# xuangu-fang/Gaussian-Process-Slover-for-High-Freq-PDE

Hardware: AMD Instinct MI355X
Metric: log-joint iters/sec + fp64 Cholesky GFLOP/s, 2D Poisson 256^2, 1-8 GPU (higher is better)
Workload: dtype f64; 1 GPU; C4: 2D Poisson 256x256 Kronecker grid, Matern52_Cos_1d, Q=30, fp64; Q=30, kernel=Matern52_Cos_1d, equation=poisson_2d-sin_sin, parallelism=replicas x1 (one independent problem per GPU)

## Files before the change

### gaussian-process-slover-for-high-freq-pde_amd/csrc/gpk_internal.h

```cpp
#pragma once
#include <vector>
#include <hip/hip_runtime.h>
#include <stdint.h>

namespace gpk {

constexpr int QMAX = 64;
constexpr int PADM = 32;
constexpr int NB = 32;
constexpr double SQRT5 = 2.23606797749978969641;
constexpr double TWO_PI = 6.28318530717958647692;

enum Kind { SE_COS = 0, MATERN52_COS = 1, SE = 2, MATERN52 = 3 };

__host__ __device__ inline bool kind_matern(int k) { return k == MATERN52_COS || k == MATERN52; }
__host__ __device__ inline bool kind_cos(int k) { return k == SE_COS || k == MATERN52_COS; }
inline int pad_up(int n) { return (n + PADM - 1) / PADM * PADM; }

struct AxisConst {
  double w[QMAX];
  double a[QMAX];
  double om[QMAX];
  double oml[QMAX];
};

__host__ __device__ inline double om_low(double freq, double om) { return fma(TWO_PI, freq, -om); }

__device__ __forceinline__ void phase_sincos(double om, double oml, double d, double& S, double& C) {
  const double h = om * d;
  const double l = fma(om, d, -h) + oml * d;
  double s, c;
  sincos(h, &s, &c);
  S = fma(l, c, s);
  C = fma(-l, s, c);
}

template <bool MATERN>
__device__ __forceinline__ double radial_exp(double d, double a, double& r) {
  double l;
  if (MATERN) {
    const double p = SQRT5 * a;
    r = p * d;
    l = fma(p, d, -r) + fma(SQRT5, a, -p) * d;
  } else {
    const double d2 = d * d;
    r = a * d2;
    l = fma(a, d2, -r) + a * fma(d, d, -d2);
  }
  const double E = exp(-r);
  return fma(-l, E, E);
}

struct StepScalars {
  double tau, v;
  double bc1, bc2;
};

template <bool MATERN>
__device__ __forceinline__ void radial(double d, double a, double& m0, double& m1, double& m2) {
  double r;
  const double E = radial_exp<MATERN>(d, a, r);
  if (MATERN) {
    m0 = (1.0 + r + r * r * (1.0 / 3.0)) * E;
    m1 = -(SQRT5 / 3.0) * a * r * (1.0 + r) * E;
    m2 = (5.0 / 3.0) * a * a * (r * r - r - 1.0) * E;
  } else {
    const double d2 = d * d, g = E;
    m0 = g;
    m1 = -2.0 * a * d * g;
    m2 = (4.0 * a * a * d2 - 2.0 * a) * g;
  }
}

template <bool MATERN>
__device__ __forceinline__ void radial_l(double d, double a, double& m0, double& m1, double& m2,
                                         double& m0l, double& m1l, double& m2l) {
  double r;
  const double E = radial_exp<MATERN>(d, a, r);
  if (MATERN) {
    double ka = (SQRT5 / 3.0) * a, k2 = (5.0 / 3.0) * a * a;
    double r2 = r * r;
    m0 = (1.0 + r + r2 * (1.0 / 3.0)) * E;
    m1 = -ka * r * (1.0 + r) * E;
    m2 = k2 * (r2 - r - 1.0) * E;
    m0l = -(r2 * (1.0 / 3.0)) * (1.0 + r) * E;
    m1l = -ka * r * (2.0 + 2.0 * r - r2) * E;
    m2l = k2 * (-r2 * r + 5.0 * r2 - 2.0 * r - 2.0) * E;
  } else {
    const double d2 = d * d, g = E;
    m0 = g;
    m1 = -2.0 * a * d * g;
    m2 = (4.0 * a * a * d2 - 2.0 * a) * g;
    m0l = -a * d2 * g;
    m1l = (-2.0 * a * d + 2.0 * a * a * d2 * d) * g;
    m2l = (10.0 * a * a * d2 - 2.0 * a - 4.0 * a * a * a * d2 * d2) * g;
  }
}

}

namespace gpk {

constexpr int BGAP_CHUNK = 2048, BGAP_PARTS_MAX = 16;
struct PrepArgs {
  const double* params;
  int off_kp[2];
  int off_tau, off_v;
  int naxes, has_cos;
  AxisConst* kc;
  StepScalars* sc;
  int* count;
  int apply;
  double b1, b2;
  const double* Up; const double* bvals; const int* bidx;
  int nb, dim, n1, n2, p2;
  double* bgap;
  int bgap_parts;
  int skip;
  int* snap_count; unsigned int* viol0; int* slot0;
  double* snap; const double* snap_m; const double* snap_v; size_t snap_np;
  unsigned int* nce_flag;
};

constexpr int CLS_VMAX = 32;
struct ClassArgs {
  int ncls;
  int vmax;
  const double* dist;
  const int* cid;
  const int* cbase;
  const unsigned char* vidx;
  double* kval;
  double* dval;
  int nchunk, rb;
  double* part;
};

struct AssembleArgs {
  const double* x;
  int n;
  int p;
  const AxisConst* kc;
  double jitter;
  double* K;
  double* Kc;
  double* D;
  int deriv;
  double* piv; double* ldet; double* pst; int* status;
  unsigned int* flag;
  ClassArgs cls;
};
hipError_t launch_gather_only(const AssembleArgs* a, int naxes, hipStream_t s);
hipError_t launch_assemble(int kind, int q, const AssembleArgs* a, int naxes, const PrepArgs& prep,
                           hipStream_t s, bool eval_only = false);
hipError_t launch_pairs(int kind, int q, const double* x1, const double* x2, long n,
                        const AxisConst* kc, int deriv, double* out, hipStream_t s);
hipError_t launch_cross(int kind, int q, const double* xr, int nr, const double* xc, int nc,
                        int ld, const AxisConst* kc, double jitter, int deriv, double* K,
                        double* D, hipStream_t s);

struct SpdArgs {
  double* X;
  double* Y;
  int p;
  int n;
  double* piv;
  double* ldet;
  double* pst;
  int* status;
  unsigned int* flag;
  int wide;
  int no_quarters;
  int qfirst;
  double* Z;
  const unsigned* sched;
  int sched_paired;
};
int wide_sched_stride(int T2);
void wide_schedule(int T2, bool paired, std::vector<unsigned>& tab);
hipError_t launch_spd_inverse(SpdArgs* args, int nmat, double** final_out, hipStream_t s,
                              bool pivot0_done = false);
hipError_t launch_spd_stage(SpdArgs* args, int nmat, int stage, hipStream_t s);

constexpr int CHAIN_MAX_BLOCKS = 512;
struct ChainArgs {
  double* X; double* PB; double* piv; double* ldet; double* pst; int* status;
  unsigned int* flags;
  int p, n;
  const int* cid; const double* kval; const double* dval; const double* x; double jitter;
  double* Kc; double* D;
  int tu, td;
  const double* Bu; int ldbu, bu_t;
  double* Ou; int ldou, ou_t;
  double* Od; int ldod;
  double* PBa; int ldpba;
  double* gran;
  int lookahead;
  double* PB2; unsigned int* epoch;
};
__host__ __device__ inline size_t multi_half(int p) { return (size_t)p * p + (size_t)32 * p; }
__host__ __device__ inline size_t chain_half(int p, bool multi) { return multi ? multi_half(p) : (size_t)32 * p; }
constexpr unsigned long long CHAIN_SENTINEL = 0x7ff4dead7ff4deadull;
constexpr unsigned int CHAIN_SENTINEL32 = 0x7ff4deadu;
int spd_chain_blocks(const int* p, int nmat, bool aug);
int spd_chain_capacity(int deriv, bool gather);
__host__ __device__ inline int chain_role(int m, int x, int T, int TC) {
  const int nt = T * TC, nc = 2 * (T - 1);
  auto crit = [TC](int i) { return (i & 1) ? ((i >> 1) + 1) * (TC + 1) : (i >> 1) * (TC + 1) + 1; };
  int r;
  if (m == 0) {
    if (x == nt) return nt;
    if (x >= nt - nc) return crit(x - (nt - nc));
    r = x;
  } else {
    if (x == 0) return nt;
    if (x <= nc) return crit(x - 1);
    r = x - 1 - nc;
  }
  int tile = r;
  for (int i = 0; i < nc; ++i)
    if (crit(i) <= tile) ++tile;
  return tile;
}
int spd_chain_multi_blocks(const int* p, int nmat);
int spd_chain_multi_capacity(int deriv, bool gather);
hipError_t launch_spd_chain_multi(const ChainArgs* a, int nmat, int deriv, hipStream_t s,
                                  const PrepArgs* prep = nullptr, int q = 0);
hipError_t launch_spd_chain(const ChainArgs* a, int nmat, int deriv, hipStream_t s,
                            const PrepArgs* prep = nullptr, int q = 0);

constexpr int SPD_BIG_MIN = 1600;
constexpr int SPD_WIDE_MIN = 3072;
size_t spd_big_piv_doubles(int p);
void spd_big_set_workgroups(int g);
constexpr unsigned SPIN_CAP = 1u << 22;
hipError_t wait_limit_spdinv(unsigned polls);
hipError_t wait_limit_spdbig(unsigned polls);
hipError_t wait_limit_assemble(unsigned polls);
hipError_t wait_limit_pgrad(unsigned polls);
hipError_t launch_spd_inverse_big(SpdArgs* args, int nmat, double** final_out, hipStream_t s);
hipError_t launch_spd_big_stage(SpdArgs* args, int nmat, int stage, hipStream_t s, bool mirror = true);
double spd_big_update_flops(const SpdArgs* args, int nmat, int k, bool with_pivot);
hipError_t launch_spd_big_tiles(SpdArgs* args, int nmat, int k, hipStream_t s);
int spd_big_sweeps(int p, int wide);

constexpr double REFINE_COND_LB = 100.0;

enum Epi {
  EPI_STORE = 0,
  EPI_RESID = 1,
  EPI_QUAD = 2,
};
struct GemmDesc {
  const double* A; const double* B; int lda, ldb, ta, tb;
  const double* A2; const double* B2; int lda2, ldb2, ta2, tb2;
  double alpha, alpha2, beta;
  const double* C0; int ldc0;
  double* C; int ldc;
  int M, N, K, K2;
  int epi;
  int ac;
  const double* F; const double* U; int ldf;
  int vscale, vscale2;
  double* red;
  double* red2; const double* Q1; const double* Q2;
  const double* gate; int ngate;
  double* Y; const double* Ys; int ldy;
  int tag;
  const double* Cp; int ldcp;
  double* cpart; const int* bcid; const int* bcbase; const double* bsx; int bn, bncls;
};
__host__ __device__ inline int class_slots(int T) { return 4 * T; }
constexpr int CB_SLOTS = 31 * 8;
constexpr int CB_VMAX = 16;
constexpr int GEMM_MAX_BATCH = 4;
struct GemmBatch {
  GemmDesc d[GEMM_MAX_BATCH];
};
hipError_t launch_gemm_batch(const GemmDesc* descs, int ndesc, int max_tiles,
                             const StepScalars* sc, hipStream_t s, int small);
inline bool gemm_use_small(long tiles16_total) { return tiles16_total <= 16384; }
enum { GEMM_TILED32 = 0, GEMM_SMALL = 1, GEMM_BIG = 2, GEMM_HUGE = 3 };
constexpr long GEMM_HUGE_MIN_TILES = 256;
int gemm_variant(const GemmDesc* descs, int ndesc, int force_big);
int gemm_tiles(const GemmDesc& d, int variant);
hipError_t launch_gemm_auto(const GemmDesc* descs, int ndesc, const StepScalars* sc, hipStream_t s,
                            int variant);

struct SlabGemm {
  const double* A; const double* B; size_t sB;
  double* C; size_t sC;
  const double* C0; size_t sC0;
  int M, N, K, nb;
  double alpha, beta;
};
constexpr int SLAB_TILE64_MIN = 512;
int slab_gemm_tile(const SlabGemm& g);
hipError_t launch_gemm_slab(const SlabGemm& g, hipStream_t s, int tile = 0);

__device__ __forceinline__ bool gate_open(const double* gate) {
  if (!gate) return true;
  const double k00 = gate[0];
  const double mx = __longlong_as_double(*reinterpret_cast<const long long*>(gate + 1));
  return mx * k00 > REFINE_COND_LB;
}

struct GemvDesc {
  const double* A; int lda; const double* x; double* y; int p; int rows;
  double alpha;
  const double* C0; double beta;
  int epi;
  int ac;
  const double* F; const double* U;
  const double* U0;
  double* red;
  double* red2; const double* Q1; const double* Q2;
  const double* gate; int ngate;
  const int* cid; const double* cv; double cdiag; int ident;
};
hipError_t launch_gemv(const GemvDesc& d, hipStream_t s);
int gemv_blocks(int rows);

struct PGradArgs {
  const double* x; int n; int p;
  const AxisConst* kc;
  const double* GK; const double* GD;
  const double* Kinv;
  const double* alpha; const double* beta; const double* R;
  double halfc;
  int deriv;
  double* part;
  double* part_lo;
  ClassArgs cls;
  const double* cpK; const double* cpD; int cslots;
};
struct TailArgs;
hipError_t launch_pgrad(int kind, int q, int mode1d, const PGradArgs* a, int naxes,
                        int blocks_per_axis, const StepScalars* sc, hipStream_t s,
                        const TailArgs* tail = nullptr, int shard_rank = 0, int shard_n = 1);
int pgrad_blocks(int n);
int pgrad_class_blocks(int ncls);

}
```

### gaussian-process-slover-for-high-freq-pde_amd/csrc/pgrad.hip

```cpp
#include <algorithm>

#include "gpk_internal.h"
#include "gpk_trace.h"
#include "fields_dd.h"
#include "spd_pivot.h"
#include "prep_dev.h"

namespace gpk {
GPK_TRACE_TU(pgrad)
GPK_WAIT_LIMIT_SETTER(wait_limit_pgrad)
}
#define FIN_PROBE(slot) TR_HI(slot)
#include "stepk_dev.h"

#ifndef GPK_PG_PAIRS
#define GPK_PG_PAIRS 64
#endif

namespace gpk {

constexpr int PAIRS = GPK_PG_PAIRS;
constexpr int PG_SUB = 1024 / PAIRS;

struct PGradBatch {
  PGradArgs ax[2];
  int tiles[2];
  int naxes, bpa;
  int shard_rank, shard_n;
  TailArgs tail;
};

__device__ __forceinline__ void st_wt(double* p, double v) {
  __hip_atomic_store(p, v, __ATOMIC_RELAXED, __HIP_MEMORY_SCOPE_AGENT);
}

__device__ __forceinline__ bool arrive_last(unsigned int* counter, unsigned int n, int* s_flag) {
  asm volatile("s_waitcnt vmcnt(0)" ::: "memory");
  __syncthreads();
  if (threadIdx.x == 0) {
    const unsigned prev = atomicAdd(counter, 1u);
    *s_flag = prev == n - 1u;
  }
  __syncthreads();
  return *s_flag != 0;
}


__device__ void pgrad_tail(const PGradBatch& b, int axis, int blk, int q) {
  const TailArgs& T = b.tail;
  __shared__ int s_last;
  const int t = threadIdx.x;
  const int gi = blk / T.tg;
  const int gsize = min(T.tg, b.bpa - gi * T.tg);
  if (t == 0 && blk == 0 && axis == 0) TR_HI(SLOT_PG_CONTRACT);
  if (t == 0 && blk == b.bpa - 1 && axis == b.naxes - 1) TR_HI(SLOT_PG_START);
  if (!arrive_last(T.gcount + axis * T.ngpa + gi, (unsigned)gsize, &s_last)) return;
  if (t == 0) {
    TR_LO(SLOT_PG_GARR);
    TR_HI(SLOT_PG_GARR);
  }
  const double* part = b.ax[axis].part;
  const double* part_lo = b.ax[axis].part_lo;
  for (int x = t; x < 3 * QMAX; x += 256) {
    const size_t go = (size_t)(axis * T.ngpa + gi) * (3 * QMAX) + x;
    if (T.gpart_lo) {
      dd::D acc = {0.0, 0.0};
      if ((x % QMAX) < q)
        acc = strided_sum_dd(part + (size_t)gi * T.tg * (3 * QMAX) + x,
                             part_lo + (size_t)gi * T.tg * (3 * QMAX) + x, 3 * QMAX, gsize);
      st_wt(T.gpart + go, acc.h);
      st_wt(T.gpart_lo + go, acc.l);
      continue;
    }
    double acc = 0.0;
    if ((x % QMAX) < q)
      acc = strided_sum(part + (size_t)gi * T.tg * (3 * QMAX) + x, 3 * QMAX, gsize);
    st_wt(T.gpart + go, acc);
  }
  if (t == 0) T.gcount[axis * T.ngpa + gi] = 0u;
  if (t == 0) TR_HI(SLOT_PG_GROUP);
  if (!arrive_last(T.top, (unsigned)(b.naxes * T.ngpa), &s_last)) return;
  if (t == 0) TR_LO(SLOT_PG_TOP);
  if (t == 0) *T.top = 0u;
  if (t == 0) TR_HI(SLOT_PG_TOP);
  finalize_body(T.fin, 2);
  if (t == 0) TR_HI(SLOT_PG_FINAL);
  if (T.nce_flag) {
    asm volatile("s_waitcnt vmcnt(0)" ::: "memory");
    __syncthreads();
    if (t == 0) __hip_atomic_store(T.nce_flag, 1u, __ATOMIC_RELAXED, __HIP_MEMORY_SCOPE_AGENT);
  }
}

template <bool MATERN, bool COS, int DERIV>
__device__ void next_class_values(const PGradBatch& b, int ax, int blk, int q) {
  const ClassArgs& C = b.ax[ax].cls;
  if (blk * 8 >= C.ncls) return;
  __shared__ double sw[QMAX], sa[QMAX], so[QMAX], sol[QMAX];
  const int t = threadIdx.x, u = blk * 8 + (t >> 5);
  const double d = u < C.ncls ? C.dist[u] : 0.0;
  if (t == 0) (void)spin_until_ge<1>(b.tail.nce_flag, 1u, b.tail.nce_status);
  __syncthreads();
  if (t < q) {
    const Layout& L = b.tail.fin.L;
    const double* kp = b.tail.fin.kp_wt + ((ax == 0 ? L.off_kp[0] : L.off_kp[1]) - L.off_small);
    axis_component_v(ld_wt(kp + t), ld_wt(kp + q + t), ld_wt(kp + 2 * q + t), sw[t], sa[t], so[t], sol[t]);
  }
  __syncthreads();
  class_value_store<MATERN, COS, DERIV>(C, u, d, sw, sa, so, sol, q);
}

template <int V, int DERIV, bool MODE1D, bool LDSB = false>
__global__ __launch_bounds__(256) void class_sum_kernel(PGradBatch b,
                                                       const StepScalars* __restrict__ sc, int vb = 0) {
  const int axis = blockIdx.z, band = blockIdx.y, chunk = blockIdx.x;
  const PGradArgs& A = b.ax[axis];
  const ClassArgs& C = A.cls;
  const int n = A.n, p = A.p;
  if (band * 64 >= n || chunk >= C.nchunk) return;
  if (MODE1D && min(n, chunk * C.rb + C.rb) - 1 < band * 64) return;
  const int t = threadIdx.x, lane = t & 63, w = t >> 6;
  if (TR_FIRST) TR_LO(SLOT_CLASS_SUM);
  if (TR_LAST) TR_LO(SLOT_CSUM_START);
  const int k = band * 64 + lane;
  const bool kv = k < n;
  const int cb = kv ? C.cbase[k] : 0;
  const int nvar = kv ? C.cbase[k + 1] - cb : 0;
  const int r0 = chunk * C.rb, r1 = min(n, r0 + C.rb);
  int nvw = V;
  if constexpr (V > 16) {
    nvw = nvar;
#pragma unroll
    for (int o = 32; o > 0; o >>= 1) nvw = max(nvw, __shfl_xor(nvw, o, 64));
    nvw = __builtin_amdgcn_readfirstlane(nvw);
  }
  double ak[LDSB ? 1 : V], ad[LDSB ? 1 : V];
#pragma unroll
  for (int x = 0; x < (LDSB ? 1 : V); ++x) ak[x] = ad[x] = 0.0;
  extern __shared__ double lbin[];
  double* mybin = lbin + (size_t)w * 2 * vb * 64;
  if constexpr (LDSB) {
    for (int x = 0; x < vb; ++x) {
      mybin[x * 64 + lane] = 0.0;
      mybin[(vb + x) * 64 + lane] = 0.0;
    }
  }
  double vs = 0.0, hc = 0.0;
  if (MODE1D) {
    vs = sc->v;
    hc = A.halfc;
  }
  static_assert(!(MODE1D && DERIV == 1), "the 1D fold assumes a symmetric G_D sign");
  constexpr int RP = MODE1D ? 8 : 4, NP = 8;
  for (int base = r0; base < r1; base += 4 * RP) {
    int ii[NP], jj[NP], msk[NP];
    if (MODE1D) {
#pragma unroll
      for (int s = 0; s < NP; ++s) {
        const int r = base + w + 4 * s;
        const bool lo = kv && r < r1 && r >= k;
        ii[s] = lo ? r : 0;
        jj[s] = lo ? r - k : 0;
        msk[s] = -(int)lo;
      }
    } else {
#pragma unroll
      for (int s = 0; s < RP; ++s) {
        const int r = base + w + 4 * s;
        const bool in = kv && r < r1;
        const bool lo = in && r >= k, up = in && k > 0 && r + k < n;
        ii[2 * s] = lo ? r : 0;
        jj[2 * s] = lo ? r - k : 0;
        msk[2 * s] = -(int)lo;
        ii[2 * s + 1] = up ? r : 0;
        jj[2 * s + 1] = up ? r + k : 0;
        msk[2 * s + 1] = -(int)up;
      }
    }
    int cv[NP];
    double g0[NP], g1[NP];
#pragma unroll
    for (int s = 0; s < NP; ++s) cv[s] = C.cid[(size_t)ii[s] * p + jj[s]];
    if (MODE1D) {
      double ai[NP], aj[NP], bi[NP], bj[NP], ri[NP], rj[NP];
#pragma unroll
      for (int s = 0; s < NP; ++s) {
        g0[s] = A.Kinv[(size_t)ii[s] * p + jj[s]];
        ai[s] = A.alpha[ii[s]];
        aj[s] = A.alpha[jj[s]];
        bi[s] = A.beta[ii[s]];
        bj[s] = A.beta[jj[s]];
        ri[s] = A.R[ii[s]];
        rj[s] = A.R[jj[s]];
      }
      if (k == 0) {
#pragma unroll
        for (int s = 0; s < NP; ++s) {
          g1[s] = vs * ri[s] * aj[s];
          g0[s] = hc * g0[s] - 0.5 * ai[s] * aj[s] - vs * bi[s] * aj[s];
        }
      } else {
#pragma unroll
        for (int s = 0; s < NP; ++s) {
          g1[s] = vs * (ri[s] * aj[s] + rj[s] * ai[s]);
          g0[s] = 2.0 * hc * g0[s] - ai[s] * aj[s] - vs * (bi[s] * aj[s] + bj[s] * ai[s]);
        }
      }
    } else {
#pragma unroll
      for (int s = 0; s < NP; ++s) g0[s] = A.GK[(size_t)ii[s] * p + jj[s]];
#pragma unroll
      for (int s = 0; s < NP; ++s) g1[s] = A.GD[(size_t)ii[s] * p + jj[s]];
    }
    if (DERIV == 1) {
      double xi[NP], xj[NP];
#pragma unroll
      for (int s = 0; s < NP; ++s) {
        xi[s] = A.x[ii[s]];
        xj[s] = A.x[jj[s]];
      }
#pragma unroll
      for (int s = 0; s < NP; ++s)
        if (!(xi[s] - xj[s] >= 0.0)) g1[s] = -g1[s];
    }
    if constexpr (LDSB) {
#pragma unroll
      for (int s = 0; s < NP; ++s) {
        const int v = cv[s] - cb;
        if (msk[s] && v >= 0 && v < vb) {
          __hip_atomic_fetch_add(mybin + v * 64 + lane, g0[s], __ATOMIC_RELAXED, __HIP_MEMORY_SCOPE_WORKGROUP);
          __hip_atomic_fetch_add(mybin + (vb + v) * 64 + lane, g1[s], __ATOMIC_RELAXED, __HIP_MEMORY_SCOPE_WORKGROUP);
        }
      }
    } else if constexpr (V > 16) {
      int vv[8];
#pragma unroll
      for (int s = 0; s < 8; ++s) vv[s] = ((cv[s] - cb) & msk[s]) | ~msk[s];
#pragma unroll
      for (int x = 0; x < V; ++x) {
        if (x < nvw) {
#pragma unroll
          for (int s = 0; s < 8; ++s) {
            ak[x] += (vv[s] == x) ? g0[s] : 0.0;
            ad[x] += (vv[s] == x) ? g1[s] : 0.0;
          }
        }
      }
    } else {
#pragma unroll
      for (int s = 0; s < 8; ++s) {
        const int v = ((cv[s] - cb) & msk[s]) | ~msk[s];
#pragma unroll
        for (int x = 0; x < V; ++x) {
          ak[x] += (v == x) ? g0[s] : 0.0;
          ad[x] += (v == x) ? g1[s] : 0.0;
        }
      }
    }
  }
  if constexpr (LDSB) {
    __syncthreads();
    if (w == 0) {
      double* pk = C.part + (size_t)chunk * C.ncls + cb;
      double* pd = C.part + (size_t)(C.nchunk + chunk) * C.ncls + cb;
      for (int x = 0; x < nvar; ++x) {
        double rk = lbin[x * 64 + lane], rd = lbin[(vb + x) * 64 + lane];
#pragma unroll
        for (int ww = 1; ww < 4; ++ww) {
          rk = rk + lbin[(size_t)ww * 2 * vb * 64 + x * 64 + lane];
          rd = rd + lbin[(size_t)ww * 2 * vb * 64 + (vb + x) * 64 + lane];
        }
        pk[x] = rk;
        pd[x] = rd;
      }
    }
    if (TR_FIRST) TR_HI(SLOT_CLASS_SUM);
    if (TR_LAST) TR_HI(SLOT_CSUM_START);
    return;
  }
  __shared__ double red[2][V][64];
#pragma unroll
  for (int ww = 0; ww < 4; ++ww) {
    if (w == ww) {
#pragma unroll
      for (int x = 0; x < V; ++x) {
        if (x < nvw) {
          red[0][x][lane] = ww == 0 ? ak[x] : red[0][x][lane] + ak[x];
          red[1][x][lane] = ww == 0 ? ad[x] : red[1][x][lane] + ad[x];
        }
      }
    }
    __syncthreads();
  }
  if (w == 0) {
    double* pk = C.part + (size_t)chunk * C.ncls + cb;
    double* pd = C.part + (size_t)(C.nchunk + chunk) * C.ncls + cb;
#pragma unroll
    for (int x = 0; x < V; ++x)
      if (x < nvar) {
        pk[x] = red[0][x][lane];
        pd[x] = red[1][x][lane];
      }
  }
  if (TR_FIRST) TR_HI(SLOT_CLASS_SUM);
  if (TR_LAST) TR_HI(SLOT_CSUM_START);
}

constexpr int PG_CLS = 16;

template <bool MATERN, bool COS, int DERIV, bool MODE1D, bool CLS, bool DD = false>
__global__ __launch_bounds__(256) void pgrad_kernel(PGradBatch b, int q,
                                                    const StepScalars* __restrict__ sc) {
  const int axis = blockIdx.y;
  const int blk = blockIdx.x;
  if (TR_FIRST) TR_LO(SLOT_PGRAD);
  if (axis == b.naxes + 1) {
    if (blk == 0) finalize_body(b.tail.fin, 1);
    return;
  }
  if (axis >= b.naxes + 2) {
    if (CLS && b.tail.nce_flag) next_class_values<MATERN, COS, DERIV>(b, axis - (b.naxes + 2), blk, q);
    return;
  }
  if (axis == b.naxes) {
    if (threadIdx.x == 0 && blk == 0) TR_LO(SLOT_PG_UPLANE);
    const int nu = tail_nu(b.tail.adam.L);
    for (int e = blk * 256 + threadIdx.x; e < nu; e += gridDim.x * 256) adam_u_elem(b.tail.adam, e);
    if (threadIdx.x == 0 && blk == 0) TR_HI(SLOT_PG_UPLANE);
    if (threadIdx.x == 0 && blk == gridDim.x - 1) TR_HI(SLOT_PG_ULAST);
    return;
  }
  if (blk >= b.bpa) return;
  const bool trl = threadIdx.x == 0 && blk == b.bpa - 1 && axis == b.naxes - 1;
  if (trl) TR_LO(SLOT_PG_START);
  const PGradArgs& A = b.ax[axis];
  const int tile = CLS ? blk : blk / PG_SUB, chunk = blk % PG_SUB;
  if (CLS ? blk * PG_CLS >= A.cls.ncls : tile >= b.tiles[axis]) {
    if (b.tail.fused) pgrad_tail(b, axis, blk, q);
    return;
  }
  if (b.shard_n > 1 && tile % b.shard_n != b.shard_rank) return;

  __shared__ double sd[PAIRS], swk[PAIRS], swd[PAIRS];
  __shared__ double sw[QMAX], sa[QMAX], so[QMAX], sol[QMAX];
  __shared__ double sacc[8][3][32];
  const int t = threadIdx.x;
  if (t < q) {
    sw[t] = A.kc->w[t];
    sa[t] = A.kc->a[t];
    so[t] = A.kc->om[t];
    sol[t] = A.kc->oml[t];
  }
  constexpr int NP = CLS ? PG_CLS : PAIRS;
  if (CLS) {
    const ClassArgs& C = A.cls;
    const int ul = t & (PG_CLS - 1), cs = t / PG_CLS;
    const int u = blk * PG_CLS + ul;
    double sk = 0.0, sdd = 0.0;
    if (u < C.ncls && A.cpK) {
      for (int e = cs; e < A.cslots; e += 256 / PG_CLS) {
        sk += A.cpK[(size_t)e * C.ncls + u];
        sdd += A.cpD[(size_t)e * C.ncls + u];
      }
    } else if (u < C.ncls) {
      for (int c = cs; c < C.nchunk; c += 256 / PG_CLS) {
        sk += C.part[(size_t)c * C.ncls + u];
        sdd += C.part[(size_t)(C.nchunk + c) * C.ncls + u];
      }
    }
    sacc[cs >> 1][0][(cs & 1) * PG_CLS + ul] = sk;
    sacc[cs >> 1][1][(cs & 1) * PG_CLS + ul] = sdd;
    __syncthreads();
    if (t < PG_CLS) {
      double a = 0.0, d = 0.0;
#pragma unroll
      for (int x = 0; x < 256 / PG_CLS; ++x) {
        a += sacc[x >> 1][0][(x & 1) * PG_CLS + t];
        d += sacc[x >> 1][1][(x & 1) * PG_CLS + t];
      }
      const bool ok = u < C.ncls;
      sd[t] = ok ? C.dist[u] : 0.0;
      swk[t] = ok ? a : 0.0;
      swd[t] = ok ? d : 0.0;
    }
  } else if (t < PAIRS) {
    int I = (int)((sqrt(8.0 * tile + 1.0) - 1.0) * 0.5);
    while ((I + 1) * (I + 2) / 2 <= tile) ++I;
    while (I * (I + 1) / 2 > tile) --I;
    const int J = tile - I * (I + 1) / 2;
    const int i = I * 32 + chunk * (PAIRS / 32) + (t >> 5), j = J * 32 + (t & 31);
    double d = 0.0, wk = 0.0, wd = 0.0;
    if (i < A.n && j < A.n) {
      const double diff = A.x[i] - A.x[j];
      d = fabs(diff);
      const double sij = diff >= 0.0 ? 1.0 : -1.0;
      const double sji = (A.x[j] - A.x[i]) >= 0.0 ? 1.0 : -1.0;
      double gkij, gkji, gdij, gdji;
      if (MODE1D) {
        const double v = sc->v;
        const double ai = A.alpha[i], aj = A.alpha[j];
        gkij = A.halfc * A.Kinv[(size_t)i * A.p + j] - 0.5 * ai * aj - v * A.beta[i] * aj;
        gkji = A.halfc * A.Kinv[(size_t)j * A.p + i] - 0.5 * aj * ai - v * A.beta[j] * ai;
        gdij = v * A.R[i] * aj;
        gdji = v * A.R[j] * ai;
      } else {
        gkij = A.GK[(size_t)i * A.p + j];
        gkji = A.GK[(size_t)j * A.p + i];
        gdij = A.GD[(size_t)i * A.p + j];
        gdji = A.GD[(size_t)j * A.p + i];
      }
      if (DERIV == 1) {
        gdij *= sij;
        gdji *= sji;
      }
      if (I == J) {
        wk = gkij;
        wd = gdij;
      } else {
        wk = gkij + gkji;
        wd = gdij + gdji;
      }
    }
    sd[t] = d;
    swk[t] = wk;
    swd[t] = wd;
  }
  __syncthreads();
  if (TR_FIRST) TR_HI(SLOT_PG_STAGED);

  const int g = t >> 5, ql = t & 31;
  double* out = A.part + (size_t)blk * (3 * QMAX);
  __shared__ double slo[DD ? 8 : 1][3][32];
  for (int q0 = 0; q0 < q; q0 += 32) {
    const int c = q0 + ql;
    double accf = 0.0, accl = 0.0, accw = 0.0;
    dd::D xf = {0.0, 0.0}, xl = {0.0, 0.0}, xw = {0.0, 0.0};
    if (c < q) {
      const double a = sa[c], om = so[c], oml = sol[c];
      for (int e = g; e < NP; e += 8) {
        const double wk = swk[e], wd = swd[e];
        if (wk == 0.0 && wd == 0.0) continue;
        const double d = sd[e];
        if constexpr (DD) {
          dd::D fw, fl, ff, dw, dl, df;
          fields_dd<MATERN, COS, DERIV>(d, a, om, oml, fw, fl, ff, dw, dl, df);
          xw = dd::add(xw, dd::add(dd::mul_d(fw, wk), dd::mul_d(dw, wd)));
          xl = dd::add(xl, dd::add(dd::mul_d(fl, wk), dd::mul_d(dl, wd)));
          xf = dd::add(xf, dd::add(dd::mul_d(ff, wk), dd::mul_d(df, wd)));
          continue;
        }
        double m0, m1, m2, m0l, m1l, m2l;
        radial_l<MATERN>(d, a, m0, m1, m2, m0l, m1l, m2l);
        if (COS) {
          double S, C;
          phase_sincos(om, oml, d, S, C);
          const double c0 = C, c1 = -om * S, c2 = -om * om * C;
          const double c0f = -TWO_PI * d * S;
          const double c1f = -TWO_PI * S - TWO_PI * om * d * C;
          const double c2f = -2.0 * TWO_PI * om * C + TWO_PI * om * om * d * S;
          double fw = m0 * c0, fl = m0l * c0, ff = m0 * c0f;
          double dw, dl, df;
          if (DERIV == 2) {
            dw = m2 * c0 + 2.0 * m1 * c1 + m0 * c2;
            dl = m2l * c0 + 2.0 * m1l * c1 + m0l * c2;
            df = m2 * c0f + 2.0 * m1 * c1f + m0 * c2f;
          } else {
            dw = m1 * c0 + m0 * c1;
            dl = m1l * c0 + m0l * c1;
            df = m1 * c0f + m0 * c1f;
          }
          accw += wk * fw + wd * dw;
          accl += wk * fl + wd * dl;
          accf += wk * ff + wd * df;
        } else {
          const double dw = DERIV == 2 ? m2 : m1, dl = DERIV == 2 ? m2l : m1l;
          accw += wk * m0 + wd * dw;
          accl += wk * m0l + wd * dl;
        }
      }
    }
    if constexpr (DD) {
      sacc[g][0][ql] = xf.h;
      sacc[g][1][ql] = xl.h;
      sacc[g][2][ql] = xw.h;
      slo[g][0][ql] = xf.l;
      slo[g][1][ql] = xl.l;
      slo[g][2][ql] = xw.l;
    } else {
      sacc[g][0][ql] = accf;
      sacc[g][1][ql] = accl;
      sacc[g][2][ql] = accw;
    }
    __syncthreads();
    if (t < 96) {
      const int which = t >> 5, qq = t & 31;
      if constexpr (DD) {
        dd::D s = {0.0, 0.0};
#pragma unroll
        for (int gg = 0; gg < 8; ++gg) s = dd::add(s, dd::D{sacc[gg][which][qq], slo[gg][which][qq]});
        if (q0 + qq < QMAX) {
          st_wt(out + which * QMAX + q0 + qq, s.h);
          st_wt(A.part_lo + (size_t)blk * (3 * QMAX) + which * QMAX + q0 + qq, s.l);
        }
      } else {
        double s = 0.0;
#pragma unroll
        for (int gg = 0; gg < 8; ++gg) s += sacc[gg][which][qq];
        if (q0 + qq < QMAX) {
          if (b.tail.fused) st_wt(out + which * QMAX + q0 + qq, s);
          else out[which * QMAX + q0 + qq] = s;
        }
      }
    }
    __syncthreads();
  }
  if (b.tail.fused) pgrad_tail(b, axis, blk, q);
}

int pgrad_blocks(int n) {
  int T = pad_up(n) / 32;
  return T * (T + 1) / 2 * PG_SUB;
}

int pgrad_class_blocks(int ncls) { return (ncls + PG_CLS - 1) / PG_CLS; }

template <int V>
static void launch_csum_v(const PGradBatch& b, int nchunk, int nbands, int deriv, int mode1d,
                          const StepScalars* sc, hipStream_t s) {
  dim3 grid(nchunk, nbands, b.naxes);
  if (mode1d)
    hipLaunchKernelGGL((class_sum_kernel<V, 2, true>), grid, dim3(256), 0, s, b, sc);
  else if (deriv == 2)
    hipLaunchKernelGGL((class_sum_kernel<V, 2, false>), grid, dim3(256), 0, s, b, sc);
  else
    hipLaunchKernelGGL((class_sum_kernel<V, 1, false>), grid, dim3(256), 0, s, b, sc);
}

static void launch_csum_lds(const PGradBatch& b, int nchunk, int nbands, int deriv, int mode1d, int vmax,
                            const StepScalars* sc, hipStream_t s) {
  dim3 grid(nchunk, nbands, b.naxes);
  const size_t lds = (size_t)4 * 2 * vmax * 64 * sizeof(double);
  if (mode1d)
    hipLaunchKernelGGL((class_sum_kernel<1, 2, true, true>), grid, dim3(256), lds, s, b, sc, vmax);
  else if (deriv == 2)
    hipLaunchKernelGGL((class_sum_kernel<1, 2, false, true>), grid, dim3(256), lds, s, b, sc, vmax);
  else
    hipLaunchKernelGGL((class_sum_kernel<1, 1, false, true>), grid, dim3(256), lds, s, b, sc, vmax);
}

template <bool MATERN, bool COS, bool CLS>
static void launch_pg_c(const PGradBatch& b, int naxes, int bpa, int q, int deriv, int mode1d,
                        const StepScalars* sc, hipStream_t s) {
  const int ublocks = b.tail.fused ? (tail_nu(b.tail.adam.L) + 255) / 256 : 0;
  dim3 grid(std::max(bpa, std::min(ublocks, 4096)), naxes + (b.tail.fused ? 2 : 0));
  if (b.tail.fused && b.tail.nce_flag) {
    for (int k = 0; k < naxes; ++k) grid.x = std::max<unsigned>(grid.x, (b.ax[k].cls.ncls + 7) / 8);
    grid.y += naxes;
  }
  const bool ddc = CLS && b.tail.fused && b.tail.gpart_lo && b.ax[0].part_lo && (naxes < 2 || b.ax[1].part_lo);
  if (ddc) {
    if (mode1d)
      hipLaunchKernelGGL((pgrad_kernel<MATERN, COS, 2, true, CLS, true>), grid, dim3(256), 0, s, b, q, sc);
    else if (deriv == 2)
      hipLaunchKernelGGL((pgrad_kernel<MATERN, COS, 2, false, CLS, true>), grid, dim3(256), 0, s, b, q, sc);
    else
      hipLaunchKernelGGL((pgrad_kernel<MATERN, COS, 1, false, CLS, true>), grid, dim3(256), 0, s, b, q, sc);
    return;
  }
  if (mode1d) {
    hipLaunchKernelGGL((pgrad_kernel<MATERN, COS, 2, true, CLS>), grid, dim3(256), 0, s, b, q, sc);
  } else if (deriv == 2) {
    hipLaunchKernelGGL((pgrad_kernel<MATERN, COS, 2, false, CLS>), grid, dim3(256), 0, s, b, q, sc);
  } else {
    hipLaunchKernelGGL((pgrad_kernel<MATERN, COS, 1, false, CLS>), grid, dim3(256), 0, s, b, q, sc);
  }
}

template <bool MATERN, bool COS>
static void launch_pg_t(const PGradBatch& b, int naxes, int bpa, int q, int deriv, int mode1d,
                        const StepScalars* sc, hipStream_t s) {
  if (b.ax[0].cls.ncls > 0) {
    int nbands = 0, vmax = 0, nchunk = 0;
    for (int k = 0; k < naxes; ++k) {
      nbands = std::max(nbands, (b.ax[k].n + 63) / 64);
      vmax = std::max(vmax, b.ax[k].cls.vmax);
      nchunk = std::max(nchunk, b.ax[k].cls.nchunk);
    }
    if (!b.ax[0].cpK) {
      if (vmax <= 8) launch_csum_v<8>(b, nchunk, nbands, deriv, mode1d, sc, s);
      else launch_csum_lds(b, nchunk, nbands, deriv, mode1d, vmax, sc, s);
    }
    launch_pg_c<MATERN, COS, true>(b, naxes, bpa, q, deriv, mode1d, sc, s);
  } else {
    launch_pg_c<MATERN, COS, false>(b, naxes, bpa, q, deriv, mode1d, sc, s);
  }
}

hipError_t launch_pgrad(int kind, int q, int mode1d, const PGradArgs* a, int naxes,
                        int blocks_per_axis, const StepScalars* sc, hipStream_t s,
                        const TailArgs* tail, int shard_rank, int shard_n) {
  PGradBatch b{};
  b.shard_rank = shard_rank;
  b.shard_n = shard_n;
  if (shard_n > 1 && tail && tail->fused) return hipErrorInvalidValue;
  for (int k = 0; k < naxes; ++k) {
    b.ax[k] = a[k];
    int T = a[k].p / 32;
    b.tiles[k] = T * (T + 1) / 2;
    if ((a[k].cls.ncls > 0) != (a[0].cls.ncls > 0) || a[k].cls.vmax > CLS_VMAX) return hipErrorInvalidValue;
    if ((a[k].cpK != nullptr) != (a[0].cpK != nullptr) ||
        (a[k].cpK && (!a[k].cpD || a[k].cslots <= 0 || a[k].cls.ncls <= 0 || mode1d)))
      return hipErrorInvalidValue;
  }
  b.naxes = naxes;
  b.bpa = blocks_per_axis;
  if (tail) b.tail = *tail;
  if (b.tail.fused) {
    if (b.tail.tg <= 0 || b.tail.ngpa * b.tail.tg < blocks_per_axis) return hipErrorInvalidValue;
  }
  if (b.tail.nce_flag && (!b.tail.fused || !b.tail.nce_status || !b.tail.fin.kp_wt || a[0].cls.ncls <= 0 ||
                          shard_n > 1))
    return hipErrorInvalidValue;
  int deriv = a[0].deriv;
  switch (kind) {
    case SE_COS: launch_pg_t<false, true>(b, naxes, blocks_per_axis, q, deriv, mode1d, sc, s); break;
    case MATERN52_COS: launch_pg_t<true, true>(b, naxes, blocks_per_axis, q, deriv, mode1d, sc, s); break;
    case SE: launch_pg_t<false, false>(b, naxes, blocks_per_axis, q, deriv, mode1d, sc, s); break;
    default: launch_pg_t<true, false>(b, naxes, blocks_per_axis, q, deriv, mode1d, sc, s); break;
  }
  return hipGetLastError();
}

}
```

Baseline: 10510 iters/s.

## Overlap class-sum loads with transcendental evaluation in class-mode pgrad kernel

In class-mode pgrad (not DD), each thread now loads its two class distances and kernel constants early. It computes exp and sincos for the first q-chunk while the batched partial-sum global loads are in flight, with scheduling barriers and asm pins holding the order. The inner pair loop is replaced by exactly two pairs per thread (g and g+8) using the precomputed transcendentals. This is meant to hide global load latency behind math. The cost is more registers and duplicated code paths.

New measurement: 10660 iters/s (median of 6 runs). +1.4%, better.

```diff
diff --git a/gaussian-process-slover-for-high-freq-pde_amd/csrc/gpk_internal.h b/gaussian-process-slover-for-high-freq-pde_amd/csrc/gpk_internal.h
--- a/gaussian-process-slover-for-high-freq-pde_amd/csrc/gpk_internal.h
+++ b/gaussian-process-slover-for-high-freq-pde_amd/csrc/gpk_internal.h
@@ -36,8 +36,7 @@
 }
 
 template <bool MATERN>
-__device__ __forceinline__ double radial_exp(double d, double a, double& r) {
-  double l;
+__device__ __forceinline__ void radial_arg(double d, double a, double& r, double& l) {
   if (MATERN) {
     const double p = SQRT5 * a;
     r = p * d;
@@ -47,6 +46,11 @@
     r = a * d2;
     l = fma(a, d2, -r) + a * fma(d, d, -d2);
   }
+}
+template <bool MATERN>
+__device__ __forceinline__ double radial_exp(double d, double a, double& r) {
+  double l;
+  radial_arg<MATERN>(d, a, r, l);
   const double E = exp(-r);
   return fma(-l, E, E);
 }
@@ -73,10 +77,8 @@
 }
 
 template <bool MATERN>
-__device__ __forceinline__ void radial_l(double d, double a, double& m0, double& m1, double& m2,
-                                         double& m0l, double& m1l, double& m2l) {
-  double r;
-  const double E = radial_exp<MATERN>(d, a, r);
+__device__ __forceinline__ void radial_l_of(double d, double a, double r, double E, double& m0, double& m1,
+                                            double& m2, double& m0l, double& m1l, double& m2l) {
   if (MATERN) {
     double ka = (SQRT5 / 3.0) * a, k2 = (5.0 / 3.0) * a * a;
     double r2 = r * r;
@@ -95,6 +97,13 @@
     m1l = (-2.0 * a * d + 2.0 * a * a * d2 * d) * g;
     m2l = (10.0 * a * a * d2 - 2.0 * a - 4.0 * a * a * a * d2 * d2) * g;
   }
+}
+template <bool MATERN>
+__device__ __forceinline__ void radial_l(double d, double a, double& m0, double& m1, double& m2,
+                                         double& m0l, double& m1l, double& m2l) {
+  double r;
+  const double E = radial_exp<MATERN>(d, a, r);
+  radial_l_of<MATERN>(d, a, r, E, m0, m1, m2, m0l, m1l, m2l);
 }
 
 }
diff --git a/gaussian-process-slover-for-high-freq-pde_amd/csrc/pgrad.hip b/gaussian-process-slover-for-high-freq-pde_amd/csrc/pgrad.hip
--- a/gaussian-process-slover-for-high-freq-pde_amd/csrc/pgrad.hip
+++ b/gaussian-process-slover-for-high-freq-pde_amd/csrc/pgrad.hip
@@ -308,6 +308,63 @@
 
 constexpr int PG_CLS = 16;
 
+struct PgTrans {
+  double E, S, C;
+};
+struct PgFields {
+  double fw, fl, ff, dw, dl, df;
+};
+template <bool MATERN, bool COS>
+__device__ __forceinline__ PgTrans pg_trans(double d, double a, double om, double oml) {
+  PgTrans t{0.0, 0.0, 0.0};
+  double r;
+  t.E = radial_exp<MATERN>(d, a, r);
+  if (COS) phase_sincos(om, oml, d, t.S, t.C);
+  return t;
+}
+template <bool MATERN, bool COS, int DERIV>
+__device__ __forceinline__ PgFields pg_fields_of(double d, double a, double om, const PgTrans& t) {
+  double r, rl, m0, m1, m2, m0l, m1l, m2l;
+  radial_arg<MATERN>(d, a, r, rl);
+  radial_l_of<MATERN>(d, a, r, t.E, m0, m1, m2, m0l, m1l, m2l);
+  PgFields f;
+  if (COS) {
+    const double S = t.S, C = t.C;
+    const double c0 = C, c1 = -om * S, c2 = -om * om * C;
+    const double c0f = -TWO_PI * d * S;
+    const double c1f = -TWO_PI * S - TWO_PI * om * d * C;
+    const double c2f = -2.0 * TWO_PI * om * C + TWO_PI * om * om * d * S;
+    f.fw = m0 * c0, f.fl = m0l * c0, f.ff = m0 * c0f;
+    if (DERIV == 2) {
+      f.dw = m2 * c0 + 2.0 * m1 * c1 + m0 * c2;
+      f.dl = m2l * c0 + 2.0 * m1l * c1 + m0l * c2;
+      f.df = m2 * c0f + 2.0 * m1 * c1f + m0 * c2f;
+    } else {
+      f.dw = m1 * c0 + m0 * c1;
+      f.dl = m1l * c0 + m0l * c1;
+      f.df = m1 * c0f + m0 * c1f;
+    }
+  } else {
+    f.fw = m0, f.fl = m0l, f.ff = 0.0;
+    f.dw = DERIV == 2 ? m2 : m1, f.dl = DERIV == 2 ? m2l : m1l, f.df = 0.0;
+  }
+  return f;
+}
+template <bool MATERN, bool COS, int DERIV>
+__device__ __forceinline__ PgFields pg_fields(double d, double a, double om, double oml) {
+  return pg_fields_of<MATERN, COS, DERIV>(d, a, om, pg_trans<MATERN, COS>(d, a, om, oml));
+}
+__device__ __forceinline__ void pg_pin(PgTrans& t) {
+  asm volatile("" : "+v"(t.E), "+v"(t.S), "+v"(t.C));
+}
+template <bool COS>
+__device__ __forceinline__ void pg_weigh(const PgFields& f, double wk, double wd, double& accw,
+                                         double& accl, double& accf) {
+  accw += wk * f.fw + wd * f.dw;
+  accl += wk * f.fl + wd * f.dl;
+  if (COS) accf += wk * f.ff + wd * f.df;
+}
+
 template <bool MATERN, bool COS, int DERIV, bool MODE1D, bool CLS, bool DD = false>
 __global__ __launch_bounds__(256) void pgrad_kernel(PGradBatch b, int q,
                                                     const StepScalars* __restrict__ sc) {
@@ -345,14 +402,79 @@
   __shared__ double sw[QMAX], sa[QMAX], so[QMAX], sol[QMAX];
   __shared__ double sacc[8][3][32];
   const int t = threadIdx.x;
-  if (t < q) {
+  constexpr bool EARLY = CLS && !DD && !(!MATERN && COS && DERIV == 1);
+  if (!EARLY && t < q) {
     sw[t] = A.kc->w[t];
     sa[t] = A.kc->a[t];
     so[t] = A.kc->om[t];
     sol[t] = A.kc->oml[t];
   }
   constexpr int NP = CLS ? PG_CLS : PAIRS;
-  if (CLS) {
+  const int g = t >> 5, ql = t & 31;
+  [[maybe_unused]] PgTrans ta{}, tb{};
+  [[maybe_unused]] double da = 0.0, db = 0.0;
+  if constexpr (EARLY) {
+    const ClassArgs& C = A.cls;
+    const int ul = t & (PG_CLS - 1), cs = t / PG_CLS;
+    const int u = blk * PG_CLS + ul;
+    const int ua = blk * PG_CLS + g, ub = ua + 8;
+    da = C.dist[min(ua, C.ncls - 1)];
+    db = C.dist[min(ub, C.ncls - 1)];
+    const int cq = max(min(ql, q - 1), 0);
+    const double a0 = A.kc->a[cq], om0 = A.kc->om[cq], oml0 = A.kc->oml[cq];
+    const int tq = min(t, QMAX - 1);
+    const double ka = A.kc->a[tq], ko = A.kc->om[tq], kol = A.kc->oml[tq];
+    const double* pK = A.cpK ? A.cpK : C.part;
+    const double* pD = A.cpK ? A.cpD : C.part + (size_t)C.nchunk * C.ncls;
+    const int ne = A.cpK ? A.cslots : C.nchunk;
+    const int uc = min(u, C.ncls - 1);
+    constexpr int SL = 256 / PG_CLS;
+    double sk = 0.0, sdd = 0.0;
+    for (int e0 = cs; e0 == cs || e0 < ne; e0 += 4 * SL) {
+      double vk[4], vd[4];
+#pragma unroll
+      for (int j = 0; j < 4; ++j) {
+        const size_t o = (size_t)min(e0 + SL * j, ne - 1) * C.ncls + uc;
+        vk[j] = pK[o];
+        vd[j] = pD[o];
+      }
+      if (e0 == cs) {
+        __builtin_amdgcn_sched_barrier(0);
+        asm volatile("" : "+v"(da), "+v"(db));
+        ta = pg_trans<MATERN, COS>(da, a0, om0, oml0);
+        tb = pg_trans<MATERN, COS>(db, a0, om0, oml0);
+        pg_pin(ta);
+        pg_pin(tb);
+#pragma unroll
+        for (int j = 0; j < 4; ++j) asm volatile("" : "+v"(vk[j]), "+v"(vd[j]));
+      }
+#pragma unroll
+      for (int j = 0; j < 4; ++j)
+        if (u < C.ncls && e0 + SL * j < ne) {
+          sk += vk[j];
+          sdd += vd[j];
+        }
+    }
+    if (t < q) {
+      sa[t] = ka;
+      so[t] = ko;
+      sol[t] = kol;
+    }
+    sacc[cs >> 1][0][(cs & 1) * PG_CLS + ul] = sk;
+    sacc[cs >> 1][1][(cs & 1) * PG_CLS + ul] = sdd;
+    __syncthreads();
+    if (t < PG_CLS) {
+      double a = 0.0, d = 0.0;
+#pragma unroll
+      for (int x = 0; x < SL; ++x) {
+        a += sacc[x >> 1][0][(x & 1) * PG_CLS + t];
+        d += sacc[x >> 1][1][(x & 1) * PG_CLS + t];
+      }
+      const bool ok = u < C.ncls;
+      swk[t] = ok ? a : 0.0;
+      swd[t] = ok ? d : 0.0;
+    }
+  } else if (CLS) {
     const ClassArgs& C = A.cls;
     const int ul = t & (PG_CLS - 1), cs = t / PG_CLS;
     const int u = blk * PG_CLS + ul;
@@ -428,14 +550,26 @@
   __syncthreads();
   if (TR_FIRST) TR_HI(SLOT_PG_STAGED);
 
-  const int g = t >> 5, ql = t & 31;
   double* out = A.part + (size_t)blk * (3 * QMAX);
   __shared__ double slo[DD ? 8 : 1][3][32];
   for (int q0 = 0; q0 < q; q0 += 32) {
     const int c = q0 + ql;
     double accf = 0.0, accl = 0.0, accw = 0.0;
     dd::D xf = {0.0, 0.0}, xl = {0.0, 0.0}, xw = {0.0, 0.0};
-    if (c < q) {
+    if constexpr (EARLY) {
+      if (c < q) {
+        const double a = sa[c], om = so[c];
+        if (q0) {
+          ta = pg_trans<MATERN, COS>(da, a, om, sol[c]);
+          tb = pg_trans<MATERN, COS>(db, a, om, sol[c]);
+        }
+        const double wka = swk[g], wda = swd[g], wkb = swk[g + 8], wdb = swd[g + 8];
+        if (!(wka == 0.0 && wda == 0.0))
+          pg_weigh<COS>(pg_fields_of<MATERN, COS, DERIV>(da, a, om, ta), wka, wda, accw, accl, accf);
+        if (!(wkb == 0.0 && wdb == 0.0))
+          pg_weigh<COS>(pg_fields_of<MATERN, COS, DERIV>(db, a, om, tb), wkb, wdb, accw, accl, accf);
+      }
+    } else if (c < q) {
       const double a = sa[c], om = so[c], oml = sol[c];
       for (int e = g; e < NP; e += 8) {
         const double wk = swk[e], wd = swd[e];
@@ -449,34 +583,7 @@
           xf = dd::add(xf, dd::add(dd::mul_d(ff, wk), dd::mul_d(df, wd)));
           continue;
         }
-        double m0, m1, m2, m0l, m1l, m2l;
-        radial_l<MATERN>(d, a, m0, m1, m2, m0l, m1l, m2l);
-        if (COS) {
-          double S, C;
-          phase_sincos(om, oml, d, S, C);
-          const double c0 = C, c1 = -om * S, c2 = -om * om * C;
-          const double c0f = -TWO_PI * d * S;
-          const double c1f = -TWO_PI * S - TWO_PI * om * d * C;
-          const double c2f = -2.0 * TWO_PI * om * C + TWO_PI * om * om * d * S;
-          double fw = m0 * c0, fl = m0l * c0, ff = m0 * c0f;
-          double dw, dl, df;
-          if (DERIV == 2) {
-            dw = m2 * c0 + 2.0 * m1 * c1 + m0 * c2;
-            dl = m2l * c0 + 2.0 * m1l * c1 + m0l * c2;
-            df = m2 * c0f + 2.0 * m1 * c1f + m0 * c2f;
-          } else {
-            dw = m1 * c0 + m0 * c1;
-            dl = m1l * c0 + m0l * c1;
-            df = m1 * c0f + m0 * c1f;
-          }
-          accw += wk * fw + wd * dw;
-          accl += wk * fl + wd * dl;
-          accf += wk * ff + wd * df;
-        } else {
-          const double dw = DERIV == 2 ? m2 : m1, dl = DERIV == 2 ? m2l : m1l;
-          accw += wk * m0 + wd * dw;
-          accl += wk * m0l + wd * dl;
-        }
+        pg_weigh<COS>(pg_fields<MATERN, COS, DERIV>(d, a, om, oml), wk, wd, accw, accl, accf);
       }
     }
     if constexpr (DD) {
```
